# nquach/TEE_optical_flow

Hardware: AMD Instinct MI355X
Metric: frame-pairs/sec @512x512 DualTVL1 (higher is better)
Workload: dtype f32

## Files before the change

include/teeflow.h:

```cpp
#ifndef TEEFLOW_H
#define TEEFLOW_H

#include <stddef.h>
#include <stdint.h>

#ifdef __cplusplus
extern "C" {
#endif

#define TF_ABI_VERSION 2

enum {
    TF_OK = 0,
    TF_ERR_INVALID_ARG = 1,
    TF_ERR_UNSUPPORTED = 2,
    TF_ERR_HIP = 3,
    TF_ERR_NOMEM = 4,
    TF_ERR_NO_DEVICE = 5
};

enum { TF_ALGO_TVL1 = 0, TF_ALGO_DEEPFLOW = 1  };

enum { TF_VARIANT_CPU = 0, TF_VARIANT_CUDA = 1 };

// ... 235 lines not shown
int tf_dbg_f16_round(tf_handle* h, const float* in, size_t n, float scale, uint16_t* out);
int tf_dbg_luma_stats(tf_handle* h, const uint8_t* rgb, int N, int H, int W, double* minmax_out, uint32_t* hist_out, double* thr_out);
void* tf_host_alloc(size_t bytes);
void  tf_host_free(void* p);
int tf_wase_compensate(tf_handle* h, float* flows, int n_flows, const uint8_t* bkgd, int n_frames, int H, int W, float scale,
                       float* background_out);
int tf_wase_compensate_device(tf_handle* h, float* flows, int n_flows, const uint8_t* bkgd, int n_frames, int H, int W, float scale,
                              float* background_out);
int tf_dbg_launch_profile(tf_handle* h, int* level, int* warp, int* it, float* ms, int max_n);
void tf_dbg_strip_rule(int n_active, int H, int RY, int slots, int* R, int* S);
int tf_dbg_pyramid(tf_handle* h, const uint8_t* img, int H, int W, int level, float* out, int* ow, int* oh);
int tf_dbg_resize(tf_handle* h, const float* src, int sw, int sh, float* dst, int dw, int dh,
                  double inv_scale_x, double inv_scale_y, float mul);
int tf_dbg_warp(tf_handle* h, const float* I0, const float* I1, const float* u1, const float* u2, int w, int hgt,
                float* I1wx, float* I1wy, float* rho_c);
int tf_dbg_median(tf_handle* h, const float* src, int w, int hgt, int ksize, float* dst);
int tf_dbg_iterate(tf_handle* h, const float* I1wx, const float* I1wy, const float* rho_c,
                   float* u1, float* u2, float* p11, float* p12, float* p21, float* p22,
                   int w, int hgt, int nsteps, int p_is_zero, unsigned long long* err_q);
int tf_dbg_stage(tf_handle* h, const float* I1wx, const float* I1wy, const float* rho_c,
                 float* u1, float* u2, float* p11, float* p12, float* p21, float* p22,
                 int B, int w, int hgt, int inner, int outer, int ksize, float thr, int variant, int p_is_zero,
                 unsigned long long* err_q, int* iters);

#ifdef __cplusplus
}
#endif
#endif
```

tee_optical_flow_amd/_lib.py:

```python
import ctypes as C
import os

from .exceptions import OpticalFlowCalculationError

_HERE = os.path.dirname(os.path.abspath(__file__))
LIB_PATH = os.environ.get("TEEFLOW_LIB", os.path.join(_HERE, "libteeflow_hip.so"))

TF_OK = 0
TF_ERR_INVALID_ARG = 1
TF_ERR_UNSUPPORTED = 2
ECHO_F16, ECHO_U8 = 0, 1
COMM_ID_BYTES = 128
HELD_SLOTS = 12
HELD_SHAPE_LEN = 5 + 2 * HELD_SLOTS
FRAMES_FORMS = {"RGB": 0, "GRAY": 1, "YBR_FULL": 2}
RLE_STAGE_BYTES = 1024
PARAM_KEYS = {
    "tau": 0, "lambda": 1, "theta": 2, "nscales": 3, "warps": 4, "epsilon": 5, "inner_iterations": 6,
    "outer_iterations": 7, "scale_step": 8, "gamma": 9, "median_filtering": 10, "use_initial_flow": 11,
}

EXPORTED_SYMBOLS = [
    "tf_abi_version", "tf_device_count", "tf_default_params", "tf_create", "tf_destroy", "tf_set_param",
    "tf_get_param", "tf_set_stream", "tf_set_profile", "tf_calc_pair", "tf_calc_seq", "tf_calc_pairs", "tf_calc_pair_f32", "tf_calc_pairs_f32",
    "tf_calc_pairs_init", "tf_calc_pairs_init_device", "tf_chain_next", "tf_calc_pairs_device", "tf_calc_seq_device", "tf_submit_pairs_device", "tf_submit_seq_device", "tf_submit_pairs", "tf_submit_seq", "tf_submit_seq_rgb", "tf_wait", "tf_condition_frames", "tf_calc_seq_rgb", "tf_saliency_frames", "tf_saliency_frames_f32", "tf_calc_seq_saliency", "tf_calc_seq_saliency_f32", "tf_clean_masks", "tf_otsu_masks", "tf_segmentor_input", "tf_segmentor_classmap", "tf_av_centroids", "tf_first_region_areas", "tf_radlong_project", "tf_radlong_project_param", "tf_polar_project_param", "tf_radlong_hist", "tf_radlong_select", "tf_radlong_overlay", "tf_radlong_shape", "tf_get_iters", "tf_last_error",
    "tf_set_tuning", "tf_dbg_counter", "tf_default_deepflow_params", "tf_create_deepflow", "tf_dbg_df_refine", "tf_dbg_df_blur", "tf_dbg_launch_profile", "tf_dbg_strip_rule", "tf_wase_compensate", "tf_wase_compensate_device", "tf_host_alloc", "tf_host_free",
    "tf_dbg_pyramid", "tf_dbg_resize", "tf_dbg_warp", "tf_dbg_median", "tf_dbg_iterate", "tf_dbg_stage", "tf_dbg_df_pyramid", "tf_dbg_df_up",
    "tf_calc_seq_rgb_f16", "tf_submit_seq_rgb_f16", "tf_calc_seq_saliency_f16", "tf_echo_frames", "tf_dbg_f16_round", "tf_dbg_luma_stats",
    "tf_calc_seq_rgb_wase", "tf_calc_seq_saliency_wase",
    "tf_calc_chains", "tf_calc_chains_device", "tf_calc_chains_rgb", "tf_dbg_chain_order",
    "tf_hold_study", "tf_hold_mask", "tf_hold_next", "tf_calc_seq_rgb_held", "tf_held_shape", "tf_release_study", "tf_held_av_centroids", "tf_held_first_region_areas",
    "tf_held_radlong_project_param", "tf_held_polar_project_param", "tf_held_radlong_overlay",
    "tf_magnitude_overlay", "tf_held_magnitude_overlay",
    "tf_inflate", "tf_hold_study_chunks", "tf_hold_mask_chunks",
    "tf_deflate", "tf_deflate_array", "tf_held_deflate",
    "tf_hold_frames", "tf_held_frames_shape", "tf_release_frames", "tf_download_frames", "tf_frames_next",
    "tf_rle_decode", "tf_hold_frames_rle", "tf_rle_stage_bytes",
    "tf_comm_unique_id", "tf_comm_init_rank", "tf_comm_init_all", "tf_allgather_flows", "tf_allgather_flows_all", "tf_comm_wait", "tf_comm_destroy",
]


class TfParams(C.Structure):
    _fields_ = [("tau", C.c_double), ("lambda_", C.c_double), ("theta", C.c_double), ("epsilon", C.c_double),
                ("scale_step", C.c_double), ("gamma", C.c_double), ("nscales", C.c_int), ("warps", C.c_int),
                ("inner_iterations", C.c_int), ("outer_iterations", C.c_int), ("median_filtering", C.c_int),
                ("use_initial_flow", C.c_int), ("algo", C.c_int), ("max_batch", C.c_int), ("variant", C.c_int)]


class TfDeepflowParams(C.Structure):
    _fields_ = [("sigma", C.c_float), ("min_size", C.c_int), ("downscale_factor", C.c_float), ("fixed_point_iterations", C.c_int),
# ... 131 lines not shown
    L.tf_inflate.argtypes = [vp, vp, vp, vp, vp, i32, C.c_uint32, vp, vp]
    L.tf_deflate.argtypes = [vp, vp, i32, C.c_uint32, vp, C.c_uint64, vp, vp, vp]
    L.tf_deflate_array.argtypes = [vp, vp, i32, vp, vp, i32, i32, vp, C.c_uint64, vp, vp, vp, vp]
    L.tf_held_deflate.argtypes = [vp, i32, i32, vp, i32, vp, C.c_uint64, vp, vp, vp, vp]
    L.tf_hold_frames.argtypes = [vp, vp, i32, i32, i32, i32, i32]
    L.tf_held_frames_shape.argtypes = [vp, C.POINTER(C.c_longlong * 4)]
    L.tf_release_frames.argtypes = [vp]
    L.tf_download_frames.argtypes = [vp, vp]
    L.tf_frames_next.argtypes = [vp, i32, i32]
    L.tf_rle_decode.argtypes = [vp, vp, vp, vp, i32, i32, i32, i32, vp, vp]
    L.tf_hold_frames_rle.argtypes = [vp, vp, vp, vp, i32, i32, i32, i32, i32, i32, vp]
    L.tf_rle_stage_bytes.restype = i32
    L.tf_hold_study_chunks.argtypes = [vp, C.POINTER(TfChunked), C.POINTER(TfChunked)]
    L.tf_hold_mask_chunks.argtypes = [vp, i32, C.POINTER(TfChunked)]
    L.tf_get_iters.argtypes = [vp, vp, C.c_size_t, C.POINTER(C.c_size_t)]
    L.tf_last_error.argtypes = [vp]
    L.tf_last_error.restype = C.c_char_p
    L.tf_dbg_pyramid.argtypes = [vp, vp, i32, i32, i32, vp, C.POINTER(i32), C.POINTER(i32)]
    L.tf_dbg_resize.argtypes = [vp, vp, i32, i32, vp, i32, i32, dbl, dbl, f32]
    L.tf_dbg_warp.argtypes = [vp, vp, vp, vp, vp, i32, i32, vp, vp, vp]
    L.tf_dbg_median.argtypes = [vp, vp, i32, i32, i32, vp]
    L.tf_dbg_iterate.argtypes = [vp] + [vp] * 9 + [i32, i32, i32, i32, vp]
    L.tf_dbg_stage.argtypes = [vp] + [vp] * 9 + [i32, i32, i32, i32, i32, i32, f32, i32, i32, vp, vp]
    L.tf_comm_unique_id.argtypes = [vp]
    L.tf_comm_init_rank.argtypes = [vp, i32, i32, vp]
    L.tf_comm_init_all.argtypes = [C.POINTER(vp), i32]
    L.tf_allgather_flows.argtypes = [vp, vp, C.c_size_t, vp, C.POINTER(i32)]
    L.tf_allgather_flows_all.argtypes = [C.POINTER(vp), i32, C.POINTER(vp), C.c_size_t, C.POINTER(vp)]
    L.tf_comm_wait.argtypes = [vp, i32]
    L.tf_comm_destroy.argtypes = [vp]
    for name in EXPORTED_SYMBOLS:
        getattr(L, name)
    if L.tf_abi_version() != 2:
        raise OpticalFlowCalculationError("libteeflow_hip.so ABI version mismatch")
    _lib = L
    return L


def check(rc, handle=None, what="teeflow"):
    if rc != TF_OK:
        msg = load().tf_last_error(handle)
        err = OpticalFlowCalculationError(f"{what} failed (code {rc}): {msg.decode() if msg else ''}")
        err.code = rc
        raise err
```

tee_optical_flow_amd/csrc/teeflow.hip:

```cpp
#include "teeflow_kernels.hip.h"
#include "teeflow_deepflow.hip.h"
#include "teeflow_sor_rt.hip.h"
#include "teeflow_analysis.hip.h"
#include "teeflow_wase.hip.h"
#include "teeflow_saliency.hip.h"
#include "teeflow_ccl.hip.h"
#include "teeflow_masks.hip.h"
#include "teeflow_otsu.hip.h"
#include "teeflow_centroid.hip.h"
#include "teeflow_area.hip.h"
#include "teeflow_polar.hip.h"
#include "teeflow_overlay.hip.h"
#include "teeflow_magoverlay.hip.h"
#include "teeflow_segmentor.hip.h"
#include "teeflow_inflate.hip.h"
#include "teeflow_deflate.hip.h"
#include "teeflow_ingest.hip.h"
#include "teeflow_rle.hip.h"
#include "pil_resample_tables.h"
#include "../../include/teeflow.h"
#include "teeflow_engine.hip.h"
#include "teeflow_tvl1_host.hip.h"
#include "teeflow_deepflow_host.hip.h"
#include "teeflow_queue.hip.h"
// ... 140 lines not shown
    else if (n == "lane_slots_pct") h->lane_slots_pct = value;
    else if (n == "strip_test_slots") h->strip_test_slots = value < 0 ? 0 : (value > (1 << 20) ? (1 << 20) : value);
    else if (n == "sor_rt") h->sor_rt = value ? 1 : 0;
    else if (n == "sor_rt_shape") h->sor_rt_shape = value;
    else if (n == "sor_plain_div") h->sor_plain_div = value ? 1 : 0;
    else if (n == "max_strip_width") h->max_strip_width = value < 4 ? 4 : (value > 2048 ? 2048 : value);
    else if (n == "lanes") h->lanes = value < 1 ? 1 : (value > 8 ? 8 : value);
    else if (n == "queue_lanes") h->queue_lanes = value;
    else if (n == "queue_unit") h->queue_unit = value < 0 ? 0 : value;
    else if (n == "queue_test_fail_unit") h->queue_test_fail_unit = value;
    else if (n == "sor_fuse") h->sor_fuse = value;
    else if (n == "sor_coop") {
        h->sor_coop = value;
        if (value) { h->coop.rearm(); ++h->sor_coop_arm; }
    }
    else if (n == "sor_coop_s") h->sor_coop_s = value;
    else if (n == "sor_coop_small") h->sor_coop_small = value ? 1 : 0;
    else if (n == "sor_coop_min_util") h->sor_coop_min_util = value;
    else if (n == "coop_test_mute") h->coop_test_mute = value ? 1 : 0;
    else if (n == "coop_test_occ16") { h->coop_test_occ16 = value; h->coop.occ16 = -1; if (h->coop.flags) h->coop.query_occupancy(*h); }
    else if (n == "coop_test_occ8") { h->coop_test_occ8 = value; h->coop.occ16 = -1; if (h->coop.flags) h->coop.query_occupancy(*h); }
    else if (n == "coop_backoff") { h->coop.backoff = value < 0 ? 0 : value; }
    else if (n == "df_fuse_ds") h->df_fuse_ds = value < 0 ? 0 : (value > 2 ? 2 : value);
    else if (n == "warp_margin") h->warp_margin = value < 0 ? 0 : (value > 40 ? 40 : value);
    else if (n == "overlay_chunk_kib") h->overlay_chunk_kib = value < 0 ? 0 : (value > (512 << 10) ? (512 << 10) : value);
    else if (n == "area_chunk_kib") h->area_chunk_kib = value < 0 ? 0 : (value > (512 << 10) ? (512 << 10) : value);
    else return fail(h, TF_ERR_INVALID_ARG, "unknown tuning knob %s", name);
    return TF_OK;
}

#ifdef TF_COOP_TIMING
extern "C" __attribute__((visibility("default"))) int tf_dbg_coop_times(unsigned long long* out)
{
    return (int)hipMemcpyFromSymbol(out, HIP_SYMBOL(g_coop_t), sizeof(unsigned long long) * 4 * 64);
}
#endif
TF_API long long tf_dbg_counter(tf_handle* h, const char* name)
{
    if (!h || !name) return -1;
    const std::string n(name);
    long long v = -1;
    for (int i = 0; i < tf_handle::DT_COUNT; ++i)
        if (n == DEV_TIME_NAMES[i]) return (long long)(h->dev_ms[i] * 1000.0);
    std::vector<CoopCounters> all{h->coop.counters()};
    if (h->pool) { std::lock_guard<std::mutex> lk(h->pool->m); all.insert(all.end(), h->pool->coop.begin(), h->pool->coop.end()); }
    if (n == "coop_launches") { v = 0; for (auto& c : all) v += c.launches; }
// ... 2 lines not shown
    else if (n == "coop_rearms") { v = 0; for (auto& c : all) v += c.rearms; }
    else if (n == "coop_cooldown") { v = 0; for (auto& c : all) v = v > c.cooldown ? v : c.cooldown; }
    else if (n == "deflate_batches") v = h->deflate_batches;
    else if (n == "queue_jobs") v = h->q_jobs;
    else if (n == "stream_retries") v = h->stream_retries;
    else if (n == "tail_upload_bytes") v = h->tail_upload_bytes;
    else if (n == "frames_upload_bytes") v = h->frames_upload_bytes;
    else if (n == "frames_held_reads") v = h->frames_held_reads;
    else if (n == "ingest_bytes") v = h->ingest_bytes;
    else if (n == "rle_bytes") v = h->rle_bytes;
    else if (n == "study_download_bytes") v = h->study_download_bytes;
    else if (n == "streams_serialised") v = h->streams_serialised;
    else if (n == "queue_units_done" || n == "queue_units_skipped" || n == "queue_units_failed" || n == "queue_outstanding" || n == "queue_lanes") {
        v = 0;
        if (h->pool) {
            std::lock_guard<std::mutex> lk(h->pool->m);
            v = n == "queue_units_done" ? h->q_units_done : n == "queue_units_skipped" ? h->q_units_skipped : n == "queue_units_failed" ? h->q_units_failed : n == "queue_outstanding" ? h->pool->outstanding : (long long)h->pool->lanes.size();
        }
    }
    else if (n == "chain_steps") {
        if (h->pool) { std::lock_guard<std::mutex> lk(h->pool->m); v = h->chain_steps; }
        else v = h->chain_steps;
    }
    else if (n == "coop_occ16") v = h->coop.occ16;
    else if (n == "coop_occ8") v = h->coop.occ8;
    return v;
}

TF_API void tf_dbg_strip_rule(int n_active, int H, int RY, int slots, int* R, int* S)
{
    int r = 0, sn = 0;
    strip_rule(n_active, H, RY, slots, &r, &sn);
    if (R) *R = r;
    if (S) *S = sn;
}

TF_API int tf_dbg_launch_profile(tf_handle* h, int* level, int* warp, int* it, float* ms, int max_n)
{
    if (!h) return -1;
    int n = 0;
    for (size_t i = 0; i < h->tally.prof_used; ++i) {
        const ProfEv& pe = h->prof_pool[i];
        if (pe.level < 0) continue;
        if (n < max_n) {
            if (level) level[n] = pe.level;
            if (warp) warp[n] = pe.warp;
// ... 149 lines not shown
```

tee_optical_flow_amd/csrc/teeflow_dbg.hip.h:

```cpp
namespace {
template <class T> struct DevBuf { T* p = nullptr; ~DevBuf() { if (p) (void)hipFree(p); } };
using DBuf = DevBuf<float>;

int dbg_up(tf_handle* h, DBuf& d, const float* src, const Geom& g)
{
    HIPC(h, hipMalloc(&d.p, (size_t)g.plane * sizeof(float)));
    HIPC(h, hipMemsetAsync(d.p, 0, (size_t)g.plane * sizeof(float), h->stream));
    if (src) HIPC(h, hipMemcpy2DAsync(d.p, (size_t)g.pitch * 4, src, (size_t)g.w * 4, (size_t)g.w * 4, g.h, hipMemcpyHostToDevice, h->stream));
    return TF_OK;
}
int dbg_down(tf_handle* h, float* dst, const float* d, const Geom& g)
{
    HIPC(h, hipMemcpy2DAsync(dst, (size_t)g.w * 4, d, (size_t)g.pitch * 4, (size_t)g.w * 4, g.h, hipMemcpyDeviceToHost, h->stream));
    HIPC(h, hipStreamSynchronize(h->stream));
    return TF_OK;
}

int dbg_up2(tf_handle* h, DBuf& fr, const float* I0, const float* I1, const Geom& g)
{
    HIPC(h, hipMalloc(&fr.p, 2 * (size_t)g.plane * sizeof(float)));
    HIPC(h, hipMemsetAsync(fr.p, 0, 2 * (size_t)g.plane * sizeof(float), h->stream));
    HIPC(h, hipMemcpy2DAsync(fr.p, (size_t)g.pitch * 4, I0, (size_t)g.w * 4, (size_t)g.w * 4, g.h, hipMemcpyHostToDevice, h->stream));
    HIPC(h, hipMemcpy2DAsync(fr.p + g.plane, (size_t)g.pitch * 4, I1, (size_t)g.w * 4, (size_t)g.w * 4, g.h, hipMemcpyHostToDevice, h->stream));
    return TF_OK;
// ... 338 lines not shown
    r.ctl = ctl.p; r.errs = errs.p; r.errstride = errstride; r.iters_dev = dit.p; r.g = g;
    r.inner = inner; r.total = total; r.ksize = ksize; r.variant = variant;
    r.thr_f = thr; r.thr_d = (double)thr;
    r.l_t = (float)(h->P.lambda * h->P.theta); r.theta = (float)h->P.theta; r.taut = (float)(h->P.tau / h->P.theta);
    r.pzero = p_is_zero ? 1 : 0;
    r.l = 0; r.wi = 0; r.nlev = 1; r.warps = 1;
    if ((rc = run_stage_loop(h, r, B))) return rc;

    std::vector<PairCtl> hc((size_t)B);
    hipError_t e = hipMemcpyAsync(hc.data(), ctl.p, (size_t)B * sizeof(PairCtl), hipMemcpyDeviceToHost, h->stream);
    if (e == hipSuccess) e = hipMemcpyAsync(err_q, errs.p, (size_t)B * errstride * sizeof(u64), hipMemcpyDeviceToHost, h->stream);
    if (e == hipSuccess) e = hipMemcpyAsync(iters, dit.p, (size_t)B * 2 * sizeof(int), hipMemcpyDeviceToHost, h->stream);
    if (e == hipSuccess) e = hipStreamSynchronize(h->stream);
    if (e != hipSuccess) return fail(h, TF_ERR_HIP, "tf_dbg_stage: %s", hipGetErrorString(e));
    for (int b = 0; b < B; ++b)
        for (int k = 0; k < 6; ++k) {
            const int half = (k < 2 ? hc[b].ubase : hc[b].pbase) & 1;
            HIPC(h, hipMemcpy2DAsync(hostp[k] + (size_t)b * hgt * w, rowb, st[2 * k + half].p + (size_t)b * g.splane, pitchb, rowb, hgt,
                                     hipMemcpyDeviceToHost, h->stream));
        }
    HIPC(h, hipStreamSynchronize(h->stream));
    return TF_OK;
}
```

tee_optical_flow_amd/csrc/teeflow_engine.hip.h:

```cpp
#include <rccl/rccl.h>
#include <algorithm>
#include <chrono>
#include <cmath>
#include <limits>
#include <cstdarg>
#include <cstdio>
#include <cstring>
#include <cstdlib>
#include <deque>
#include <string>
#include <atomic>
#include <condition_variable>
#include <mutex>
#include <thread>
#include <map>
#include <vector>

#define TF_API extern "C" __attribute__((visibility("default")))

namespace {
constexpr int MAXLEV = 64;
constexpr int DF_MAXLEV = 201;
constexpr int SLOT_RING = 1024;
constexpr int DEFAULT_LAG = 1;
// ... 1 lines not shown

thread_local std::string g_create_error;

struct ProfEv { hipEvent_t a, b; int level = 0, warp = 0, it = 0; float ms = 0.f; double work = 0.0; };
}

namespace { struct Engine; }
struct LanePool;
struct QJob;
struct CoopCounters { long long launches = 0; int aborts = 0, rearms = 0, cooldown = 0; bool disabled = false; };
struct TfKnobs {
    int iter_variant = 2;
    int max_strip_width = 2048;
    int sor_rt = 1;
    int sor_plain_div = 0;
    int sor_rt_shape = 3;
    int df_fuse_ds = 2;
    int sor_coop = 1;
    int sor_coop_min_util = 85;
    int sor_coop_small = 1;
    int sor_coop_s = 5;
    int sor_fuse = 5;
    int warp_margin = 8;
    int min_rows_work = 8192;
    int strip_blocks = 2048;
    int lane_slots_pct = 67;
    int strip_test_slots = 0;
    int coop_test_occ16 = -1, coop_test_occ8 = -1;
    int coop_test_mute = 0;
    int profile = 0;
    int overlay_chunk_kib = 0;
    int area_chunk_kib = 0;
    unsigned sor_coop_arm = 0;
};

namespace {
struct Tvl1State {
    int H = 0, W = 0, cap = 0, nlev = 0;
    double scale_step = 0; int nscales = 0, variant = 0;
    Geom lv[MAXLEV];
    float* pyr[MAXLEV] = {};
    float* gxl[MAXLEV] = {}; float* gyl[MAXLEV] = {};
    float *cwx = nullptr, *cwy = nullptr, *crho = nullptr;
    StateBufs sb = {};
    PairCtl* ctl = nullptr;
    u64* errs = nullptr; int errstride = 0;
// ... 41 lines not shown
    void release();
};

struct Engine : TfKnobs {
    tf_params P;
    tf_deepflow_params DP = {};
    int dev = 0;
    int num_cus = 256;
    hipStream_t own_stream = nullptr, stream = nullptr;
    std::string err;
    hipStream_t copy_stream = nullptr;
    hipEvent_t cev[4] = {nullptr, nullptr, nullptr, nullptr};
    uint8_t* st_u8 = nullptr; size_t st_u8_bytes = 0;
    uint8_t* st_flow = nullptr; size_t st_flow_bytes = 0;
    uint8_t* st_init = nullptr; size_t st_init_bytes = 0;
    hipEvent_t ev[4] = {};
    std::deque<ProfEv> prof_pool;
    struct Tally {
        unsigned long long iter_launches = 0;
        double df_sor_bytes = 0;
        double df_sor_px = 0;
        size_t prof_used = 0;
        long long chain_steps = 0;
    } tally;
    int slots_pct = 100;
    Tvl1State tv;
    DfState df;
    Coop coop;
};
}

struct tf_handle : Engine {
    std::vector<int> last_iters;
    struct GrowBuf { void* p = nullptr; size_t cap = 0; };
    enum { PRE_SRC, PRE_G0, PRE_G1, PRE_ION, PRE_IOFF, PRE_P, PRE_I, PRE_MON, PRE_MOFF, PRE_MX, PRE_OUT,
           PRE_LB_PAR, PRE_LB_AUX, PRE_LB_LR,
           PRE_MK_CLS, PRE_MK_OUT, PRE_MK_META,
           PRE_OT_RGB, PRE_OT_CLEAN, PRE_OT_OUT, PRE_OT_META,
           PRE_CT_MASK, PRE_CT_SUM, PRE_CT_OUT,
           PRE_AN_FLOW, PRE_AN_MASK, PRE_AN_META,
           PRE_PO_META, PRE_PO_OUT,
           PRE_AN_HIST, PRE_AN_SEL,
           PRE_OV_IDX, PRE_OV_ECHO, PRE_OV_OUT, PRE_OV_META,
           PRE_MO_IDX, PRE_MO_ECHO, PRE_MO_OUT, PRE_MO_META,
           PRE_WA_VALS, PRE_WA_CNT, PRE_WA_OFF, PRE_WA_SUM, PRE_WA_BG,
           PRE_WS_FLOW, PRE_WS_OUT,
// ... 20 lines not shown
        long long gen = 0;
        struct Mask { uint8_t* p = nullptr; int n_frames = 0, C = 0; } mask[TF_HELD_SLOTS];
        void release()
        {
            if (N) ++gen;
            (void)hipFree(flow); (void)hipFree(echo);
            for (auto& m : mask) { (void)hipFree(m.p); m = Mask(); }
            flow = echo = nullptr; N = H = W = n_echo = 0;
        }
    } held;
    struct Frames {
        uint8_t* rgb = nullptr; size_t cap = 0;
        int N = 0, H = 0, W = 0;
        long long gen = 0;
        void drop() { if (N) ++gen; N = H = W = 0; }
        void release() { drop(); (void)hipFree(rgb); rgb = nullptr; cap = 0; }
    } frames;
    long long frames_upload_bytes = 0;
    long long frames_held_reads = 0;
    long long ingest_bytes = 0;
    long long rle_bytes = 0;
    struct Armed { bool chain = false, hold = false, frames = false; int first = 0, count = 0; } armed;
    long long chain_steps = 0;
    long long study_download_bytes = 0;
    long long tail_upload_bytes = 0;
    ncclComm_t comm = nullptr; int comm_rank = 0, comm_size = 0;
    hipStream_t comm_stream = nullptr; hipEvent_t comm_ev[8] = {}; hipEvent_t comm_ready = nullptr; unsigned comm_tickets = 0;
    int lanes = 2;
    int queue_lanes = -1;
    int queue_unit = 0;
    int queue_test_fail_unit = -1;
    LanePool* pool = nullptr;
    long long q_jobs = 0, q_units_done = 0, q_units_skipped = 0, q_units_failed = 0;
    std::map<int, QJob*> tickets; int next_ticket = 1;
    int stream_retries = 0;
    int streams_serialised = 0;
};

TF_API int tf_create(const tf_params* p, int device_id, tf_handle** out);
TF_API int tf_create_deepflow(const tf_deepflow_params* p, int device_id, tf_handle** out);
TF_API const char* tf_last_error(tf_handle* h);
TF_API int tf_comm_destroy(tf_handle* h);

namespace {
constexpr tf_handle::Armed SPEND_CHAIN{true, false, false}, SPEND_FRAMES{false, false, true}, SPEND_ALL{true, true, true};

// ... 149 lines not shown
```

tee_optical_flow_amd/csrc/teeflow_kernels.hip.h:

```cpp
#pragma once
#include <hip/hip_runtime.h>
#include <stdint.h>
#include <float.h>

#define TF_HD __host__ __device__

typedef unsigned long long u64;

struct Geom {
    int w, h, pitch;
    long long plane;
    long long splane;
};

struct PairCtl {
    int ubase;
    int pbase;
};

struct StateBufs {
    float* u1[2]; float* u2[2];
    float* p11[2]; float* p12[2]; float* p21[2]; float* p22[2];
};

// ... 113 lines not shown
        if (x >= g.w || y >= g.h) return;
        const int uc = ctl[b].ubase & 1;
        const size_t i = (size_t)b * g.splane + (size_t)y * g.pitch + x;
        float2 v = make_float2(sb.u1[uc][i] * scale, sb.u2[uc][i] * scale);
        reinterpret_cast<float2*>(out)[((size_t)b * g.h + y) * g.w + x] = v;
    } else {
        if (y >= g.h) return;
        const int uc = ctl[b].ubase & 1;
        const float* u1 = sb.u1[uc] + (size_t)b * g.splane + (size_t)y * g.pitch;
        const float* u2 = sb.u2[uc] + (size_t)b * g.splane + (size_t)y * g.pitch;
        store_flow_row_f16(out + ((size_t)b * g.h + y) * g.w * 2, g.w, x, scale, [&](int px) { return make_float2(u1[px], u2[px]); });
    }
}

__global__ __launch_bounds__(256) void k_dbg_f16_round(const float* __restrict__ in, size_t n, float scale, uint16_t* __restrict__ out)
{
    const size_t i = (size_t)blockIdx.x * 256 + threadIdx.x;
    if (i < n) out[i] = (uint16_t)scaled_half_bits(in[i], scale);
}

#include "teeflow_tvl1_warp.hip.h"
#include "teeflow_tvl1_iter.hip.h"
#include "teeflow_tvl1_median.hip.h"
#include "teeflow_cond.hip.h"
```

tee_optical_flow_amd/csrc/teeflow_queue.hip.h:

```cpp
enum Mode { MODE_PAIRS, MODE_SEQ };
enum { W_HOST = 0, W_IN_DEV = 1, W_OUT_DEV = 2, W_DEV = 3 };
struct ChainSet {
    std::vector<const uint8_t*> in;
    std::vector<void*> out;
    std::vector<int> pairs;
    std::vector<int> order;
    std::vector<size_t> first;
    int count() const { return (int)pairs.size(); }
    int running(int k) const { int n = 0; while (n < count() && pairs[n] > k) ++n; return n; }
};
inline std::vector<int> chain_order(const int* n_frames, int n_chains)
{
    std::vector<int> order(n_chains > 0 ? n_chains : 0);
    for (int c = 0; c < n_chains; ++c) order[c] = c;
    std::stable_sort(order.begin(), order.end(), [&](int a, int b) { return n_frames[a] > n_frames[b]; });
    return order;
}

struct Call {
    Mode mode = MODE_PAIRS; const uint8_t* in0 = nullptr; const uint8_t* in1 = nullptr; int n_pairs = 0, H = 0, W = 0; float scale = 1.f;
    void* out = nullptr;
    int where = W_HOST;
    bool f32 = false;
    bool out_f16 = false;
// ... 384 lines not shown
        int rc = TF_OK;
        const int c0 = u * j->unit, nb = j->call.n_pairs - c0 < j->unit ? j->call.n_pairs - c0 : j->unit;
        if (!skip) {
            lane->P = j->P; lane->DP = j->DP; lane->slots_pct = j->slots_pct; lane->coop.share = share;
            if (lane->sor_coop_arm != j->knobs.sor_coop_arm) lane->coop.rearm();
            static_cast<TfKnobs&>(*lane) = j->knobs;
            if (lane->coop.flags) lane->coop.query_occupancy(*lane);
            if (u == j->fail_unit) rc = fail(lane, TF_ERR_HIP, "injected failure (queue_test_fail_unit)");
            else rc = calc_common_guarded(lane, j->call.part(c0, nb), j->iters.data() + (size_t)c0 * j->per_pair, &us);
        }
        bool last;
        {
            std::lock_guard<std::mutex> lk(pool->m);
            if (skip) ++owner->q_units_skipped; else if (rc != TF_OK) ++owner->q_units_failed; else ++owner->q_units_done;
            if (!skip && rc != TF_OK) {
                if (j->rc == TF_OK) {
                    j->rc = rc;
                    char where[96]; snprintf(where, sizeof where, "sub-batch %d (pairs %d..%d): ", u, c0, c0 + nb - 1);
                    j->err = std::string(where) + lane->err;
                }
            } else if (!skip) {
                merge_stats(&j->st, us);
                owner->chain_steps += lane->tally.chain_steps;
            }
            pool->coop[k] = lane->coop.counters();
            last = ++j->done == j->n_units;
            if (last) {
                j->finished = true;
                if (--pool->outstanding == 0 && pool->coop_held) { coop_release(lane->dev); pool->coop_held = false; }
            }
        }
        if (last) pool->cv_done.notify_all();
    }
}

void pool_destroy(tf_handle* h)
{
    LanePool* pool = h->pool;
    if (!pool) return;
    {
        std::lock_guard<std::mutex> lk(pool->m);
        pool->stop = true;
    }
    pool->cv_work.notify_all();
    for (auto& t : pool->th) t.join();
    for (Engine* l : pool->lanes) { engine_destroy(l); delete l; }
// ... 83 lines not shown

int start_call(tf_handle* h, const Call& c, QJob* j, bool submitted)
{
    const bool can_queue = queue_lane_count(h) > 0 && h->stream == h->own_stream;
    bool busy = submitted;
    if (can_queue && h->pool && !busy) { std::lock_guard<std::mutex> lk(h->pool->m); busy = h->pool->outstanding > 0; }
    const int parts = !busy && (c.chains || c.n_pairs <= sub_batch_pairs(h)) ? (c.chain ? 1 : split_count(h, c.n_pairs)) : 0;
    const bool deep = h->P.algo == TF_ALGO_DEEPFLOW;
    Geom lv[DF_MAXLEV];
    j->call = c;
    j->nlev = deep ? df_levels(h->DP, c.H, c.W, lv) : compute_levels(h->P, c.H, c.W, lv);
    j->warps = deep ? 0 : h->P.warps;
    j->per_pair = (size_t)j->nlev * j->warps * 2;
    j->iters.assign((size_t)c.n_pairs * j->per_pair, 0);
    if (can_queue && parts != 1) {
        const int rc = queue_submit(h, j, !busy, parts);
        if (rc == TF_OK) return TF_OK;
        j->rc = rc;
    } else {
        CoopClaim claim(deep ? h->dev : -1);
        h->coop.share = claim.ok ? h->num_cus : 0;
        j->t0 = now_ms();
        j->rc = calc_common_guarded(h, c, j->iters.data(), &j->st);
        if (j->rc == TF_OK && h->tally.chain_steps) {
            if (h->pool) { std::lock_guard<std::mutex> lk(h->pool->m); h->chain_steps += h->tally.chain_steps; }
            else h->chain_steps += h->tally.chain_steps;
        }
    }
    if (j->rc != TF_OK) j->err = h->err;
    j->finished = true;
    return j->rc;
}

int queue_finish(tf_handle* h, QJob* j, tf_stats* st)
{
    if (h->pool) {
        std::unique_lock<std::mutex> lk(h->pool->m);
        h->pool->cv_done.wait(lk, [&] { return j->finished; });
    }
    h->last_iters = std::move(j->iters);
    if (j->rc != TF_OK) { h->err = j->err; return j->rc; }
    if (st) {
        *st = j->st;
        st->n_pairs = j->call.n_pairs; st->nscales_used = j->nlev; st->warps = j->warps;
        st->ms_total = now_ms() - j->t0;
    }
    return TF_OK;
}

// ... 35 lines not shown
```

tee_optical_flow_amd/csrc/teeflow_tvl1_host.hip.h:

```cpp
namespace {
int validate_params(Engine* h, const tf_params& p)
{
    if (p.algo != TF_ALGO_TVL1) return fail(h, TF_ERR_UNSUPPORTED, "algo %d not implemented (only TF_ALGO_TVL1)", p.algo);
    if (p.nscales < 1 || p.nscales > MAXLEV) return fail(h, TF_ERR_INVALID_ARG, "nscales must be in [1,%d], got %d", MAXLEV, p.nscales);
    if (p.warps < 1) return fail(h, TF_ERR_INVALID_ARG, "warps must be >= 1, got %d", p.warps);
    if (p.inner_iterations < 1 || p.outer_iterations < 1)
        return fail(h, TF_ERR_INVALID_ARG, "inner/outer iterations must be >= 1, got %d/%d", p.inner_iterations, p.outer_iterations);
    if ((long long)p.inner_iterations * p.outer_iterations > 100000)
        return fail(h, TF_ERR_INVALID_ARG, "inner*outer iterations too large");
    if (p.median_filtering != 1 && p.median_filtering != 3 && p.median_filtering != 5)
        return fail(h, TF_ERR_UNSUPPORTED, "medianFiltering must be 1, 3 or 5 (cv::medianBlur on CV_32F), got %d", p.median_filtering);
    if (p.gamma != 0.0) return fail(h, TF_ERR_UNSUPPORTED, "gamma != 0 (illumination term u3) is not implemented");
    if (p.variant != TF_VARIANT_CPU && p.variant != TF_VARIANT_CUDA) return fail(h, TF_ERR_INVALID_ARG, "variant must be TF_VARIANT_CPU or TF_VARIANT_CUDA, got %d", p.variant);
    if (p.variant == TF_VARIANT_CUDA && (p.inner_iterations * p.outer_iterations) % 2 != 0)
        return fail(h, TF_ERR_UNSUPPORTED, "TF_VARIANT_CUDA needs an even iteration count (inner*outer), got %d", p.inner_iterations * p.outer_iterations);
    if (p.use_initial_flow && p.variant == TF_VARIANT_CUDA)
        return fail(h, TF_ERR_UNSUPPORTED, "useInitialFlow is not implemented for TF_VARIANT_CUDA (nothing checks that form bit for bit)");
    if (!(p.scale_step > 0.0 && p.scale_step < 1.0)) return fail(h, TF_ERR_INVALID_ARG, "scaleStep must be in (0,1), got %g", p.scale_step);
    if (p.scale_step == 0.5) return fail(h, TF_ERR_UNSUPPORTED, "scaleStep == 0.5 makes cv::resize take its INTER_AREA fast path for the pyramid, which is not implemented");
    if (!(p.theta > 0.0) || !(p.tau > 0.0) || !(p.lambda > 0.0) || !(p.epsilon >= 0.0))
        return fail(h, TF_ERR_INVALID_ARG, "tau, lambda, theta must be > 0 and epsilon >= 0");
    return TF_OK;
}

// ... 154 lines not shown
                if (hipStreamQuery(s) == hipSuccess && h->tv.slots_host[*checked % SLOT_RING] < 0)
                    return fail(h, TF_ERR_HIP, "stream drained but launch %u did not report", *checked);
            }
        }
        ++*checked;
        if (v == 0) { *stop = true; break; }
    }
    return TF_OK;
}

struct StageRun {
    const float *wx, *wy, *rho;
    StateBufs sb; PairCtl* ctl;
    u64* errs; int errstride;
    int* iters_dev;
    Geom g;
    int inner, total;
    int ksize;
    int variant;
    float thr_f; double thr_d;
    float l_t, theta, taut;
    int pzero;
    int l, wi, nlev, warps;
};

int run_stage_loop(Engine* h, const StageRun& r, int B)
{
    const Geom g = r.g;
    const int inner = r.inner, total = r.total;
    const double thr_q = (double)r.thr_f * 1073741824.0;
    hipStream_t s = h->stream;
    HIPC(h, hipMemsetAsync(r.errs, 0, (size_t)B * r.errstride * sizeof(u64), s));

    Iter2Args A;
    IterArgs& ia = A.a;
    ia.wx = r.wx; ia.wy = r.wy; ia.rho = r.rho; ia.sb = r.sb; ia.ctl = r.ctl; ia.err = r.errs;
    ia.errstride = r.errstride; ia.thr_q = thr_q; ia.g = g;
    ia.l_t = r.l_t; ia.theta = r.theta; ia.taut = r.taut;
    ia.variant = r.variant; ia.thr_d = r.thr_d;
    const bool cuda_variant = r.variant == TF_VARIANT_CUDA;
    const bool median = r.ksize > 1 && !cuda_variant;
    MedArgs ma;
    ma.sb = r.sb; ma.ctl = r.ctl; ma.err = r.errs; ma.errstride = r.errstride; ma.thr_q = thr_q; ma.g = g;

    const dim3 gm((g.w + 63) / 64, (g.h + 15) / 16, 2 * B);
    ia.B = B;
    const int step = iter_step(h, cuda_variant, inner);
    ma.total = A.total = total; ma.step = step;
    A.utog_prev = A.ptog_prev = A.pzero_prev = 0;
    int utog = 0, ptog = 0;
    bool stop = false;
    unsigned checked = h->tv.launch_seq;
    for (int it = 0; it < total + step - 1 && !stop; it += step) {
        if (it < total && it % inner == 0 && median) {
            ma.it = it; ma.utog = utog;
            int rc = profiled(h, s, -5, 0, 0, [&] {
                if (r.ksize == 5) hipLaunchKernelGGL(k_median<5>, gm, dim3(256), 0, s, ma);
                else hipLaunchKernelGGL(k_median<3>, gm, dim3(256), 0, s, ma);
            });
            if (rc) return rc;
            ++utog;
        }
        const unsigned q = h->tv.launch_seq++;
        h->tv.slots_host[q % SLOT_RING] = -1;
        ia.host_slot = h->tv.slots_dev + q % SLOT_RING;
        ia.it = it; ia.utog = utog; ia.ptog = ptog; ia.pzero = (r.pzero && it == 0) ? 1 : 0;
        int rc = profiled(h, s, r.l, r.wi, it, [&] { launch_iter(h, A, step, B, s); });
        if (rc) return rc;
        ++h->tally.iter_launches;
        A.utog_prev = utog; A.ptog_prev = ptog; A.pzero_prev = ia.pzero;
        ++utog; ++ptog;
        rc = read_reports(h, s, q, &checked, &stop);
        if (rc) return rc;
    }
    hipLaunchKernelGGL(k_stage_end, dim3((B + 255) / 256), dim3(256), 0, s, r.errs, r.errstride, r.ctl, r.iters_dev, B,
                       total, inner, median ? 1 : 0, thr_q, r.l, r.wi, r.nlev, r.warps, r.variant, r.thr_d, step);
    return TF_OK;
}

int run_stage(Engine* h, int l, int wi, int B, int off0, int off1, int* iters_dev)
{
    const tf_params& P = h->P;
    const Geom g = h->tv.lv[l];
    hipStream_t s = h->stream;

    WarpArgs wa;
    wa.pyr = h->tv.pyr[l]; wa.off0 = off0; wa.off1 = off1; wa.sb = h->tv.sb; wa.ctl = h->tv.ctl; wa.tab = h->tv.tab;
    wa.wx = h->tv.cwx; wa.wy = h->tv.cwy; wa.rho = h->tv.crho; wa.g = g;
    int rc = profiled(h, s, -4, 0, 0, [&] { launch_warp(h, wa, B, s, h->tv.gxl[l], h->tv.gyl[l]); });
    if (rc) return rc;

    StageRun r;
    r.wx = h->tv.cwx; r.wy = h->tv.cwy; r.rho = h->tv.crho; r.sb = h->tv.sb; r.ctl = h->tv.ctl;
    r.errs = h->tv.errs; r.errstride = h->tv.errstride; r.iters_dev = iters_dev; r.g = g;
    r.inner = P.inner_iterations; r.total = P.inner_iterations * P.outer_iterations;
    r.ksize = P.median_filtering; r.variant = P.variant;
    r.thr_f = (float)(P.epsilon * P.epsilon * (double)(g.w * g.h));
    r.thr_d = P.epsilon * P.epsilon * (double)(g.w * g.h);
    r.l_t = (float)(P.lambda * P.theta); r.theta = (float)P.theta; r.taut = (float)(P.tau / P.theta);
    r.pzero = wi == 0 ? 1 : 0;
    r.l = l; r.wi = wi; r.nlev = h->tv.nlev; r.warps = P.warps;
    return run_stage_loop(h, r, B);
}

void pyramids_below_level0(Engine* h, int F)
{
    const tf_params& P = h->P;
    hipStream_t s = h->stream;
    for (int l = 1; l < h->tv.nlev; ++l) {
        const double sc = 1.0 / P.scale_step;
        hipLaunchKernelGGL(k_pyr_down, grid64x4(h->tv.lv[l], F), dim3(256), 0, s, h->tv.pyr[l - 1], h->tv.lv[l - 1], h->tv.pyr[l], h->tv.lv[l], sc, sc,
                           P.variant == TF_VARIANT_CUDA ? 1 : 0);
    }
    if (P.variant == TF_VARIANT_CUDA)
        for (int l = 0; l < h->tv.nlev; ++l)
// ... 114 lines not shown
```

Baseline: 2955.

## Fuse stage warp with first median filter into a single prologue kernel

Adds a k_warp_med kernel that stages the flow tile and its halo in shared memory once. It uses that tile both to warp I1 (gradients and rho) and to write the median-filtered flow into the toggled buffer. The stage loop then skips its first median launch. The goal is to remove one kernel launch and a repeat global read of u1/u2 per warp stage. The cost is a larger shared-memory footprint and more register pressure per block. A debug entry point and tally counters are added to check it.

Result: no change. 2954 (-0.0%).

```diff
diff --git a/include/teeflow.h b/include/teeflow.h
--- a/include/teeflow.h
+++ b/include/teeflow.h
@@ -281,6 +281,8 @@
                  float* u1, float* u2, float* p11, float* p12, float* p21, float* p22,
                  int B, int w, int hgt, int inner, int outer, int ksize, float thr, int variant, int p_is_zero,
                  unsigned long long* err_q, int* iters);
+int tf_dbg_stage_prologue(tf_handle* h, const float* I0, const float* I1, float* u1, float* u2, const int* ubase,
+                          int B, int w, int hgt, int ksize, float* I1wx, float* I1wy, float* rho_c);
 
 #ifdef __cplusplus
 }
diff --git a/tee_optical_flow_amd/_lib.py b/tee_optical_flow_amd/_lib.py
--- a/tee_optical_flow_amd/_lib.py
+++ b/tee_optical_flow_amd/_lib.py
@@ -25,7 +25,7 @@
     "tf_get_param", "tf_set_stream", "tf_set_profile", "tf_calc_pair", "tf_calc_seq", "tf_calc_pairs", "tf_calc_pair_f32", "tf_calc_pairs_f32",
     "tf_calc_pairs_init", "tf_calc_pairs_init_device", "tf_chain_next", "tf_calc_pairs_device", "tf_calc_seq_device", "tf_submit_pairs_device", "tf_submit_seq_device", "tf_submit_pairs", "tf_submit_seq", "tf_submit_seq_rgb", "tf_wait", "tf_condition_frames", "tf_calc_seq_rgb", "tf_saliency_frames", "tf_saliency_frames_f32", "tf_calc_seq_saliency", "tf_calc_seq_saliency_f32", "tf_clean_masks", "tf_otsu_masks", "tf_segmentor_input", "tf_segmentor_classmap", "tf_av_centroids", "tf_first_region_areas", "tf_radlong_project", "tf_radlong_project_param", "tf_polar_project_param", "tf_radlong_hist", "tf_radlong_select", "tf_radlong_overlay", "tf_radlong_shape", "tf_get_iters", "tf_last_error",
     "tf_set_tuning", "tf_dbg_counter", "tf_default_deepflow_params", "tf_create_deepflow", "tf_dbg_df_refine", "tf_dbg_df_blur", "tf_dbg_launch_profile", "tf_dbg_strip_rule", "tf_wase_compensate", "tf_wase_compensate_device", "tf_host_alloc", "tf_host_free",
-    "tf_dbg_pyramid", "tf_dbg_resize", "tf_dbg_warp", "tf_dbg_median", "tf_dbg_iterate", "tf_dbg_stage", "tf_dbg_df_pyramid", "tf_dbg_df_up",
+    "tf_dbg_pyramid", "tf_dbg_resize", "tf_dbg_warp", "tf_dbg_median", "tf_dbg_iterate", "tf_dbg_stage", "tf_dbg_stage_prologue", "tf_dbg_df_pyramid", "tf_dbg_df_up",
     "tf_calc_seq_rgb_f16", "tf_submit_seq_rgb_f16", "tf_calc_seq_saliency_f16", "tf_echo_frames", "tf_dbg_f16_round", "tf_dbg_luma_stats",
     "tf_calc_seq_rgb_wase", "tf_calc_seq_saliency_wase",
     "tf_calc_chains", "tf_calc_chains_device", "tf_calc_chains_rgb", "tf_dbg_chain_order",
@@ -203,6 +203,7 @@
     L.tf_dbg_median.argtypes = [vp, vp, i32, i32, i32, vp]
     L.tf_dbg_iterate.argtypes = [vp] + [vp] * 9 + [i32, i32, i32, i32, vp]
     L.tf_dbg_stage.argtypes = [vp] + [vp] * 9 + [i32, i32, i32, i32, i32, i32, f32, i32, i32, vp, vp]
+    L.tf_dbg_stage_prologue.argtypes = [vp] + [vp] * 5 + [i32, i32, i32, i32, vp, vp, vp]
     L.tf_comm_unique_id.argtypes = [vp]
     L.tf_comm_init_rank.argtypes = [vp, i32, i32, vp]
     L.tf_comm_init_all.argtypes = [C.POINTER(vp), i32]
diff --git a/tee_optical_flow_amd/csrc/teeflow.hip b/tee_optical_flow_amd/csrc/teeflow.hip
--- a/tee_optical_flow_amd/csrc/teeflow.hip
+++ b/tee_optical_flow_amd/csrc/teeflow.hip
@@ -186,6 +186,7 @@
     else if (n == "coop_test_occ8") { h->coop_test_occ8 = value; h->coop.occ16 = -1; if (h->coop.flags) h->coop.query_occupancy(*h); }
     else if (n == "coop_backoff") { h->coop.backoff = value < 0 ? 0 : value; }
     else if (n == "df_fuse_ds") h->df_fuse_ds = value < 0 ? 0 : (value > 2 ? 2 : value);
+    else if (n == "stage_prologue") h->stage_prologue = value ? 1 : 0;
     else if (n == "warp_margin") h->warp_margin = value < 0 ? 0 : (value > 40 ? 40 : value);
     else if (n == "overlay_chunk_kib") h->overlay_chunk_kib = value < 0 ? 0 : (value > (512 << 10) ? (512 << 10) : value);
     else if (n == "area_chunk_kib") h->area_chunk_kib = value < 0 ? 0 : (value > (512 << 10) ? (512 << 10) : value);
@@ -234,6 +235,10 @@
         if (h->pool) { std::lock_guard<std::mutex> lk(h->pool->m); v = h->chain_steps; }
         else v = h->chain_steps;
     }
+    else if (n == "stage_prologues") {
+        if (h->pool) { std::lock_guard<std::mutex> lk(h->pool->m); v = h->stage_prologues; }
+        else v = h->stage_prologues;
+    }
     else if (n == "coop_occ16") v = h->coop.occ16;
     else if (n == "coop_occ8") v = h->coop.occ8;
     return v;
diff --git a/tee_optical_flow_amd/csrc/teeflow_dbg.hip.h b/tee_optical_flow_amd/csrc/teeflow_dbg.hip.h
--- a/tee_optical_flow_amd/csrc/teeflow_dbg.hip.h
+++ b/tee_optical_flow_amd/csrc/teeflow_dbg.hip.h
@@ -384,3 +384,64 @@
     HIPC(h, hipStreamSynchronize(h->stream));
     return TF_OK;
 }
+
+TF_API int tf_dbg_stage_prologue(tf_handle* h, const float* I0, const float* I1, float* u1, float* u2, const int* ubase,
+                                 int B, int w, int hgt, int ksize, float* I1wx, float* I1wy, float* rho_c)
+{
+    if (!h || !I0 || !I1 || !u1 || !u2 || !ubase || !I1wx || !I1wy || !rho_c) return TF_ERR_INVALID_ARG;
+    if (B < 1 || B > 4096) return fail(h, TF_ERR_INVALID_ARG, "tf_dbg_stage_prologue: B must be in [1,4096], got %d", B);
+    if (w < 1 || hgt < 1) return fail(h, TF_ERR_INVALID_ARG, "tf_dbg_stage_prologue: bad size %d x %d", w, hgt);
+    if (ksize != 0 && ksize != 1 && ksize != 3 && ksize != 5)
+        return fail(h, TF_ERR_INVALID_ARG, "tf_dbg_stage_prologue: ksize must be 0, 1, 3 or 5, got %d", ksize);
+    HIPC(h, hipSetDevice(h->dev));
+    const Geom g = make_geom(w, hgt);
+    const size_t npl = (size_t)B * (size_t)g.plane, rowb = (size_t)w * 4, pitchb = (size_t)g.pitch * 4, hostpl = (size_t)B * hgt * w;
+    DBuf fr, st[4], cst[3], dgx, dgy;
+    const auto up = [&](DBuf& d, const float* src, int n) -> int {
+        HIPC(h, hipMalloc(&d.p, n * npl * sizeof(float)));
+        HIPC(h, hipMemsetAsync(d.p, 0, n * npl * sizeof(float), h->stream));
+        if (src) HIPC(h, hipMemcpy2DAsync(d.p, pitchb, src, rowb, rowb, (size_t)n * B * hgt, hipMemcpyHostToDevice, h->stream));
+        return TF_OK;
+    };
+    int rc;
+    if ((rc = up(fr, nullptr, 2))) return rc;
+    HIPC(h, hipMemcpy2DAsync(fr.p, pitchb, I0, rowb, rowb, (size_t)B * hgt, hipMemcpyHostToDevice, h->stream));
+    HIPC(h, hipMemcpy2DAsync(fr.p + npl, pitchb, I1, rowb, rowb, (size_t)B * hgt, hipMemcpyHostToDevice, h->stream));
+    float* hostu[2] = {u1, u2};
+    for (int k = 0; k < 4; ++k) if ((rc = up(st[k], hostu[k >> 1] + (size_t)(k & 1) * hostpl, 1))) return rc;
+    for (int k = 0; k < 3; ++k) if ((rc = up(cst[k], nullptr, 1))) return rc;
+    std::vector<PairCtl> hc((size_t)B);
+    for (int b = 0; b < B; ++b) { hc[b].ubase = ubase[b]; hc[b].pbase = 0; }
+    DevBuf<PairCtl> ctl;
+    HIPC(h, hipMalloc(&ctl.p, (size_t)B * sizeof(PairCtl)));
+    HIPC(h, hipMemcpyAsync(ctl.p, hc.data(), (size_t)B * sizeof(PairCtl), hipMemcpyHostToDevice, h->stream));
+    if (h->P.variant == TF_VARIANT_CUDA) {
+        HIPC(h, hipMalloc(&dgx.p, 2 * npl * sizeof(float))); HIPC(h, hipMalloc(&dgy.p, 2 * npl * sizeof(float)));
+        hipLaunchKernelGGL(k_grad, grid64x4(g, 2 * B), dim3(256), 0, h->stream, fr.p, dgx.p, dgy.p, g);
+    }
+    WarpArgs wa = {};
+    wa.pyr = fr.p; wa.off0 = 0; wa.off1 = B; wa.ctl = ctl.p; wa.tab = h->tv.tab;
+    for (int k = 0; k < 2; ++k) { wa.sb.u1[k] = st[k].p; wa.sb.u2[k] = st[2 + k].p; }
+    wa.wx = cst[0].p; wa.wy = cst[1].p; wa.rho = cst[2].p; wa.g = g;
+    const long long before = h->tally.prologues;
+    bool med0_done = false;
+    if ((rc = run_stage_prologue(h, wa, ksize, B, dgx.p, dgy.p, &med0_done))) return rc;
+    h->stage_prologues += h->tally.prologues - before;
+    if (!med0_done && (ksize == 3 || ksize == 5) && h->P.variant == TF_VARIANT_CPU) {
+        MedArgs ma = {};
+        ma.sb = wa.sb; ma.ctl = ctl.p; ma.err = nullptr; ma.errstride = 0; ma.it = 0; ma.thr_q = 0; ma.utog = 0; ma.g = g;
+        ma.total = 1; ma.step = iter_step(h, false, h->P.inner_iterations);
+        const dim3 gm((g.w + 63) / 64, (g.h + 15) / 16, 2 * B);
+        if (ksize == 5) hipLaunchKernelGGL(k_median<5>, gm, dim3(256), 0, h->stream, ma);
+        else hipLaunchKernelGGL(k_median<3>, gm, dim3(256), 0, h->stream, ma);
+    }
+    hipError_t e = hipStreamSynchronize(h->stream);
+    if (e != hipSuccess) return fail(h, TF_ERR_HIP, "tf_dbg_stage_prologue: %s", hipGetErrorString(e));
+    float* hostc[3] = {I1wx, I1wy, rho_c};
+    for (int k = 0; k < 3; ++k)
+        HIPC(h, hipMemcpy2DAsync(hostc[k], rowb, cst[k].p, pitchb, rowb, (size_t)B * hgt, hipMemcpyDeviceToHost, h->stream));
+    for (int k = 0; k < 4; ++k)
+        HIPC(h, hipMemcpy2DAsync(hostu[k >> 1] + (size_t)(k & 1) * hostpl, rowb, st[k].p, pitchb, rowb, (size_t)B * hgt, hipMemcpyDeviceToHost, h->stream));
+    HIPC(h, hipStreamSynchronize(h->stream));
+    return TF_OK;
+}
diff --git a/tee_optical_flow_amd/csrc/teeflow_engine.hip.h b/tee_optical_flow_amd/csrc/teeflow_engine.hip.h
--- a/tee_optical_flow_amd/csrc/teeflow_engine.hip.h
+++ b/tee_optical_flow_amd/csrc/teeflow_engine.hip.h
@@ -47,6 +47,7 @@
     int sor_coop_s = 5;
     int sor_fuse = 5;
     int warp_margin = 8;
+    int stage_prologue = 1;
     int min_rows_work = 8192;
     int strip_blocks = 2048;
     int lane_slots_pct = 67;
@@ -134,6 +135,7 @@
         double df_sor_px = 0;
         size_t prof_used = 0;
         long long chain_steps = 0;
+        long long prologues = 0;
     } tally;
     int slots_pct = 100;
     Tvl1State tv;
@@ -200,6 +202,7 @@
     long long rle_bytes = 0;
     struct Armed { bool chain = false, hold = false, frames = false; int first = 0, count = 0; } armed;
     long long chain_steps = 0;
+    long long stage_prologues = 0;
     long long study_download_bytes = 0;
     long long tail_upload_bytes = 0;
     ncclComm_t comm = nullptr; int comm_rank = 0, comm_size = 0;
diff --git a/tee_optical_flow_amd/csrc/teeflow_kernels.hip.h b/tee_optical_flow_amd/csrc/teeflow_kernels.hip.h
--- a/tee_optical_flow_amd/csrc/teeflow_kernels.hip.h
+++ b/tee_optical_flow_amd/csrc/teeflow_kernels.hip.h
@@ -159,4 +159,5 @@
 #include "teeflow_tvl1_warp.hip.h"
 #include "teeflow_tvl1_iter.hip.h"
 #include "teeflow_tvl1_median.hip.h"
+#include "teeflow_tvl1_prologue.hip.h"
 #include "teeflow_cond.hip.h"
diff --git a/tee_optical_flow_amd/csrc/teeflow_queue.hip.h b/tee_optical_flow_amd/csrc/teeflow_queue.hip.h
--- a/tee_optical_flow_amd/csrc/teeflow_queue.hip.h
+++ b/tee_optical_flow_amd/csrc/teeflow_queue.hip.h
@@ -430,6 +430,7 @@
             } else if (!skip) {
                 merge_stats(&j->st, us);
                 owner->chain_steps += lane->tally.chain_steps;
+                owner->stage_prologues += lane->tally.prologues;
             }
             pool->coop[k] = lane->coop.counters();
             last = ++j->done == j->n_units;
@@ -559,9 +560,9 @@
         h->coop.share = claim.ok ? h->num_cus : 0;
         j->t0 = now_ms();
         j->rc = calc_common_guarded(h, c, j->iters.data(), &j->st);
-        if (j->rc == TF_OK && h->tally.chain_steps) {
-            if (h->pool) { std::lock_guard<std::mutex> lk(h->pool->m); h->chain_steps += h->tally.chain_steps; }
-            else h->chain_steps += h->tally.chain_steps;
+        if (j->rc == TF_OK && (h->tally.chain_steps || h->tally.prologues)) {
+            if (h->pool) { std::lock_guard<std::mutex> lk(h->pool->m); h->chain_steps += h->tally.chain_steps; h->stage_prologues += h->tally.prologues; }
+            else { h->chain_steps += h->tally.chain_steps; h->stage_prologues += h->tally.prologues; }
         }
     }
     if (j->rc != TF_OK) j->err = h->err;
diff --git a/tee_optical_flow_amd/csrc/teeflow_tvl1_host.hip.h b/tee_optical_flow_amd/csrc/teeflow_tvl1_host.hip.h
--- a/tee_optical_flow_amd/csrc/teeflow_tvl1_host.hip.h
+++ b/tee_optical_flow_amd/csrc/teeflow_tvl1_host.hip.h
@@ -200,6 +200,7 @@
     float l_t, theta, taut;
     int pzero;
     int l, wi, nlev, warps;
+    bool med0_done = false;
 };
 
 int run_stage_loop(Engine* h, const StageRun& r, int B)
@@ -226,11 +227,11 @@
     const int step = iter_step(h, cuda_variant, inner);
     ma.total = A.total = total; ma.step = step;
     A.utog_prev = A.ptog_prev = A.pzero_prev = 0;
-    int utog = 0, ptog = 0;
+    int utog = r.med0_done ? 1 : 0, ptog = 0;
     bool stop = false;
     unsigned checked = h->tv.launch_seq;
     for (int it = 0; it < total + step - 1 && !stop; it += step) {
-        if (it < total && it % inner == 0 && median) {
+        if (it < total && it % inner == 0 && median && !(it == 0 && r.med0_done)) {
             ma.it = it; ma.utog = utog;
             int rc = profiled(h, s, -5, 0, 0, [&] {
                 if (r.ksize == 5) hipLaunchKernelGGL(k_median<5>, gm, dim3(256), 0, s, ma);
@@ -256,19 +257,46 @@
     return TF_OK;
 }
 
+void launch_warp_med(Engine* h, const WarpArgs& wa, int M, int ksize, int B, hipStream_t s)
+{
+    const Geom& g = wa.g;
+    const int R = ksize / 2;
+    const dim3 grid((g.w + WL_TW - 1) / WL_TW, (g.h + WL_TH - 1) / WL_TH, B);
+    const size_t shm = (size_t)(128 + 2 * ((WL_TW + 2 * R + 3) / 4 * 4) * (WL_TH + 2 * R) + (WL_TW + 2 * (M + 4)) * (WL_TH + 2 * M + 7)) * sizeof(float);
+    switch (M * 8 + ksize) {
+        case 4 * 8 + 3: hipLaunchKernelGGL((k_warp_med<4, 3>), grid, dim3(256), shm, s, wa); break;
+        case 4 * 8 + 5: hipLaunchKernelGGL((k_warp_med<4, 5>), grid, dim3(256), shm, s, wa); break;
+        case 8 * 8 + 3: hipLaunchKernelGGL((k_warp_med<8, 3>), grid, dim3(256), shm, s, wa); break;
+        case 8 * 8 + 5: hipLaunchKernelGGL((k_warp_med<8, 5>), grid, dim3(256), shm, s, wa); break;
+        case 16 * 8 + 3: hipLaunchKernelGGL((k_warp_med<16, 3>), grid, dim3(256), shm, s, wa); break;
+        default: hipLaunchKernelGGL((k_warp_med<16, 5>), grid, dim3(256), shm, s, wa); break;
+    }
+    ++h->tally.prologues;
+}
+
+int run_stage_prologue(Engine* h, const WarpArgs& wa, int ksize, int B, const float* gx, const float* gy, bool* med0_done)
+{
+    hipStream_t s = h->stream;
+    const int M = warp_margin_class(h->warp_margin);
+    *med0_done = h->stage_prologue && h->P.variant == TF_VARIANT_CPU && (ksize == 3 || ksize == 5) && M != 0;
+    return profiled(h, s, -4, 0, 0, [&] {
+        if (*med0_done) launch_warp_med(h, wa, M, ksize, B, s);
+        else launch_warp(h, wa, B, s, gx, gy);
+    });
+}
+
 int run_stage(Engine* h, int l, int wi, int B, int off0, int off1, int* iters_dev)
 {
     const tf_params& P = h->P;
     const Geom g = h->tv.lv[l];
-    hipStream_t s = h->stream;
 
     WarpArgs wa;
     wa.pyr = h->tv.pyr[l]; wa.off0 = off0; wa.off1 = off1; wa.sb = h->tv.sb; wa.ctl = h->tv.ctl; wa.tab = h->tv.tab;
     wa.wx = h->tv.cwx; wa.wy = h->tv.cwy; wa.rho = h->tv.crho; wa.g = g;
-    int rc = profiled(h, s, -4, 0, 0, [&] { launch_warp(h, wa, B, s, h->tv.gxl[l], h->tv.gyl[l]); });
+    StageRun r;
+    int rc = run_stage_prologue(h, wa, P.median_filtering, B, h->tv.gxl[l], h->tv.gyl[l], &r.med0_done);
     if (rc) return rc;
 
-    StageRun r;
     r.wx = h->tv.cwx; r.wy = h->tv.cwy; r.rho = h->tv.crho; r.sb = h->tv.sb; r.ctl = h->tv.ctl;
     r.errs = h->tv.errs; r.errstride = h->tv.errstride; r.iters_dev = iters_dev; r.g = g;
     r.inner = P.inner_iterations; r.total = P.inner_iterations * P.outer_iterations;
diff --git a/tee_optical_flow_amd/csrc/teeflow_tvl1_prologue.hip.h b/tee_optical_flow_amd/csrc/teeflow_tvl1_prologue.hip.h
--- /dev/null
+++ b/tee_optical_flow_amd/csrc/teeflow_tvl1_prologue.hip.h
@@ -0,0 +1,149 @@
+#pragma once
+
+template <int M, int KS>
+__global__ __launch_bounds__(256) void k_warp_med(WarpArgs a)
+{
+    extern __shared__ __attribute__((aligned(16))) float smem[];
+    constexpr int R = KS / 2, LWS = WL_TW + 2 * R, LW = (LWS + 3) / 4 * 4, LH = WL_TH + 2 * R;
+    constexpr int MX = M + 4, SW = WL_TW + 2 * MX, SH = WL_TH + 2 * M + 7, QW = SW / 4, NQ = QW * SH, NV = (NQ + 255) / 256;
+    static_assert(M % 4 == 0, "margin classes are multiples of 4");
+    static_assert((LH * LW) % 4 == 0, "the staged I1 region starts on a 16-byte boundary");
+    float* stab = smem;
+    float (*t1)[LW] = reinterpret_cast<float (*)[LW]>(smem + 128);
+    float (*t2)[LW] = t1 + LH;
+    float* S = smem + 128 + 2 * LH * LW;
+    const int b = blockIdx.z;
+    const int W = a.g.w, H = a.g.h, pitch = a.g.pitch;
+    const int x0 = blockIdx.x * WL_TW, y0 = blockIdx.y * WL_TH;
+    const int rx0 = x0 - MX, ry0 = y0 - M - 3;
+    const float* __restrict__ I0 = a.pyr + (size_t)(a.off0 + b) * a.g.plane;
+    const float* __restrict__ I1 = a.pyr + (size_t)(a.off1 + b) * a.g.plane;
+    const int uc = a.ctl[b].ubase & 1;
+    const size_t po = (size_t)b * a.g.splane;
+    const float* __restrict__ s1 = a.sb.u1[uc] + po;
+    const float* __restrict__ s2 = a.sb.u2[uc] + po;
+    const int tid = threadIdx.x, lx = tid & 63, x = x0 + lx, ty = tid >> 6;
+    float i0r[4];
+#pragma unroll
+    for (int r = 0; r < 4; ++r) {
+        const int y = y0 + ty + 4 * r;
+        i0r[r] = (x < W && y < H) ? I0[(size_t)y * pitch + x] : 0.f;
+    }
+    float4 v[NV];
+#pragma unroll
+    for (int k = 0; k < NV; ++k) {
+        const int i = tid + 256 * k;
+        if (i < NQ) {
+            const int ly = i / QW, gx = rx0 + 4 * (i - ly * QW);
+            const float* row = I1 + (size_t)clampi(ry0 + ly, 0, H - 1) * pitch;
+            if (gx >= 0 && gx + 3 < W) v[k] = *reinterpret_cast<const float4*>(row + gx);
+            else v[k] = make_float4(row[clampi(gx, 0, W - 1)], row[clampi(gx + 1, 0, W - 1)], row[clampi(gx + 2, 0, W - 1)], row[clampi(gx + 3, 0, W - 1)]);
+        }
+    }
+    if (x0 + 64 <= W) {
+        constexpr int NM = (LH * 16 + 255) / 256;
+        float4 m1[NM], m2[NM];
+#pragma unroll
+        for (int k = 0; k < NM; ++k) {
+            const int i = tid + 256 * k, ly = i >> 4, q = i & 15;
+            if (i < LH * 16) {
+                const size_t o = (size_t)clampi(y0 - R + ly, 0, H - 1) * pitch + x0 + 4 * q;
+                m1[k] = *reinterpret_cast<const float4*>(s1 + o);
+                m2[k] = *reinterpret_cast<const float4*>(s2 + o);
+            }
+        }
+        const bool halo = tid < LH * 2 * R;
+        const int hly = tid / (2 * R), hc = tid % (2 * R), hlx = hc < R ? hc : 64 + hc;
+        float h1 = 0.f, h2 = 0.f;
+        if (halo) {
+            const size_t o = (size_t)clampi(y0 - R + hly, 0, H - 1) * pitch + clampi(x0 - R + hlx, 0, W - 1);
+            h1 = s1[o]; h2 = s2[o];
+        }
+        if (tid < 128) stab[tid] = a.tab[tid];
+#pragma unroll
+        for (int k = 0; k < NV; ++k) {
+            const int i = tid + 256 * k;
+            if (i < NQ) *reinterpret_cast<float4*>(S + 4 * i) = v[k];
+        }
+#pragma unroll
+        for (int k = 0; k < NM; ++k) {
+            const int i = tid + 256 * k, ly = i >> 4, q = i & 15;
+            if (i < LH * 16) {
+                float* d1 = &t1[ly][R + 4 * q];
+                float* d2 = &t2[ly][R + 4 * q];
+                if constexpr (R % 2 == 0) {
+                    *reinterpret_cast<float2*>(d1) = make_float2(m1[k].x, m1[k].y);
+                    *reinterpret_cast<float2*>(d1 + 2) = make_float2(m1[k].z, m1[k].w);
+                    *reinterpret_cast<float2*>(d2) = make_float2(m2[k].x, m2[k].y);
+                    *reinterpret_cast<float2*>(d2 + 2) = make_float2(m2[k].z, m2[k].w);
+                } else {
+                    d1[0] = m1[k].x; d1[1] = m1[k].y; d1[2] = m1[k].z; d1[3] = m1[k].w;
+                    d2[0] = m2[k].x; d2[1] = m2[k].y; d2[2] = m2[k].z; d2[3] = m2[k].w;
+                }
+            }
+        }
+        if (halo) { t1[hly][hlx] = h1; t2[hly][hlx] = h2; }
+    } else {
+        constexpr int NS = (LH * LWS + 255) / 256;
+        float sv1[NS], sv2[NS];
+#pragma unroll
+        for (int k = 0; k < NS; ++k) {
+            const int i = tid + 256 * k, ly = i / LWS, mx = i % LWS;
+            if (i < LH * LWS) {
+                const size_t o = (size_t)clampi(y0 - R + ly, 0, H - 1) * pitch + clampi(x0 - R + mx, 0, W - 1);
+                sv1[k] = s1[o]; sv2[k] = s2[o];
+            }
+        }
+        if (tid < 128) stab[tid] = a.tab[tid];
+#pragma unroll
+        for (int k = 0; k < NV; ++k) {
+            const int i = tid + 256 * k;
+            if (i < NQ) *reinterpret_cast<float4*>(S + 4 * i) = v[k];
+        }
+#pragma unroll
+        for (int k = 0; k < NS; ++k) {
+            const int i = tid + 256 * k, ly = i / LWS, mx = i % LWS;
+            if (i < LH * LWS) { t1[ly][mx] = sv1[k]; t2[ly][mx] = sv2[k]; }
+        }
+    }
+    __syncthreads();
+    if (x < W) {
+#pragma unroll
+        for (int r = 0; r < 4; ++r) {
+            const int y = y0 + ty + 4 * r;
+            if (y >= H) break;
+            const size_t idx = (size_t)y * pitch + x;
+            const float u1 = t1[ty + 4 * r + R][lx + R], u2 = t2[ty + 4 * r + R][lx + R];
+            const float mx = (float)x + u1, my = (float)y + u2;
+            const int sx = __float2int_rn(mx * 32.f), sy = __float2int_rn(my * 32.f);
+            const float* wxp = stab + (sx & 31) * 4;
+            const float* wyp = stab + (sy & 31) * 4;
+            const int ix = clampi(sx >> 5, -32768, 32767) - 1, iy = clampi(sy >> 5, -32768, 32767) - 1;
+            float vI = 0.f, vX = 0.f, vY = 0.f;
+            if (!(ix >= W || ix + 4 <= 0 || iy >= H || iy + 4 <= 0)) {
+                float P[6][6];
+                const int px = ix - 1 - rx0, py = iy - 1 - ry0;
+                if (px >= 0 && py >= 0 && px + 6 <= SW && py + 6 <= SH) {
+                    const float* Sp = S + py * SW + px;
+#pragma unroll
+                    for (int j = 0; j < 6; ++j)
+#pragma unroll
+                        for (int i = 0; i < 6; ++i) P[j][i] = Sp[j * SW + i];
+                } else {
+#pragma unroll
+                    for (int j = 0; j < 6; ++j) {
+                        const float* row = I1 + (size_t)clampi(iy - 1 + j, 0, H - 1) * pitch;
+#pragma unroll
+                        for (int i = 0; i < 6; ++i) P[j][i] = row[clampi(ix - 1 + i, 0, W - 1)];
+                    }
+                }
+                warp_accumulate(P, wxp, wyp, ix, iy, W, H, vI, vX, vY);
+            }
+            a.wx[po + idx] = vX;
+            a.wy[po + idx] = vY;
+            a.rho[po + idx] = ((vI - vX * u1) - vY * u2) - i0r[r];
+        }
+    }
+    median_tile<KS, LW>(t1, a.sb.u1[uc ^ 1] + po, x0, y0, W, H, pitch);
+    median_tile<KS, LW>(t2, a.sb.u2[uc ^ 1] + po, x0, y0, W, H, pitch);
+}
```
